# ruiminshen/yolo2-pytorch

Measured on NVIDIA H100. Metric: 416x416 images/sec, higher is better.
Workload: dtype f16

## Files before the change

yolo2-pytorch_b200/b200/engine.py:

```python
import os

import torch

from . import ops

STRICT_KEEP = {'layers1.0': 'aw', 'layers1.2': 'aw', 'layers1.4': 'a', 'passthrough': 'aw', 'layers3.0': 'aw'}
PRECISIONS = ('fast', 'strict')


class ConvUnit(object):

    def __init__(self, conv, bn, act):
        self.conv, self.bn, self.act = conv, bn, act
        self._wver = None
        self._bver = None
        self.w16 = self.scale = self.shift = None
        self.split_a = self.split_w = False
        self.out_lo = False

    @property
    def cout(self):
        return self.conv.weight.shape[0]

    @property
# ... 6 lines not shown

    @property
    def slope(self):
        return 0.1 if self.act else 1.0

    def refresh(self, first_layer=False, force=False):
        w = self.conv.weight
        wver = (w.data_ptr(), w._version)
        wver = wver + (self.split_a, self.split_w)
        if force or wver != self._wver:
            if first_layer:
                self.w16 = w.detach().contiguous()
            elif self.split_a or self.split_w:
                self.w16 = ops.pack_weight_split_f16(w.detach().contiguous(), self.split_a, self.split_w)
            else:
                self.w16 = ops.pack_weight_f16(w.detach().contiguous(), 0)
            self._wver = wver
        if self.bn is not None:
            ts = (self.bn.weight, self.bn.bias, self.bn.running_mean, self.bn.running_var)
            bver = tuple((t.data_ptr(), t._version) for t in ts)
            if bver != self._bver:
                self.scale, self.shift = ops.bn_fold(*(t.detach().contiguous() for t in ts), eps=self.bn.eps)
                self._bver = bver
        else:
            b = self.conv.bias
            bver = None if b is None else (b.data_ptr(), b._version)
            if bver != self._bver or self.scale is None:
                self.scale = torch.ones(self.cout, dtype=torch.float32, device=w.device)
                self.shift = (b.detach().float().contiguous().clone() if b is not None
                              else torch.zeros(self.cout, dtype=torch.float32, device=w.device))
                self._bver = bver


class StrictPlan(object):

    def __init__(self, eng, batch, height, width, device):
        f16 = dict(dtype=torch.float16, device=device)

        def buf(u, h, w):
            return torch.empty(batch, h, w, u.cout * (2 if u.out_lo else 1), **f16)

        h, w = height // 2, width // 2
        self.a0 = torch.empty(batch, h, w, eng.units1[0].cout, **f16)
        self.l1 = []
        for u, pooled in zip(eng.units1[1:], eng.pools1[1:]):
            out = buf(u, h, w)
            if pooled:
                h, w = h // 2, w // 2
                self.l1.append((out, buf(u, h, w)))
            else:
                self.l1.append((out, None))
        self.pt = buf(eng.unit_pt, h, w)
        h, w = h // 2, w // 2
        self.x1_pool = buf(eng.units1[-1], h, w)
        self.cat_c = eng.unit_pt.cout * 4 + eng.units2[-1].cout
        self.cat = torch.empty(batch, h, w, self.cat_c * (2 if eng.units3[0].split_a else 1), **f16)
        self.l2 = [buf(u, h, w) for u in eng.units2[:-1]]
        self.l3 = buf(eng.units3[0], h, w)
        self.feature = torch.empty(batch, eng.units3[1].cout, h, w, dtype=torch.float32, device=device)
        self.workspace = ops.conv_workspace(device)


class DarknetPlan(object):

    def __init__(self, units1, units2, unit_pt, units3, pools1, batch, height, width, device):
        f16 = dict(dtype=torch.float16, device=device)
        self.batch, self.height, self.width = batch, height, width
        h, w = height // 2, width // 2
        self.a0 = torch.empty(batch, h, w, units1[0].cout, **f16)
        self.l1 = []
        for u, pooled in zip(units1[1:], pools1[1:]):
            out = torch.empty(batch, h, w, u.cout, **f16)
            if pooled:
                h, w = h // 2, w // 2
                self.l1.append((out, torch.empty(batch, h, w, u.cout, **f16)))
            else:
                self.l1.append((out, None))
        self.h16, self.w16 = h, w
        self.pt = torch.empty(batch, h, w, unit_pt.cout, **f16)
        self.x1_pool = torch.empty(batch, h // 2, w // 2, units1[-1].cout, **f16)
        h, w = h // 2, w // 2
        self.h32, self.w32 = h, w
        self.cat_ch = unit_pt.cout * 4 + units2[-1].cout
        self.cat = torch.empty(batch, h, w, self.cat_ch, **f16)
        self.l2 = [torch.empty(batch, h, w, u.cout, **f16) for u in units2[:-1]]
        self.l3 = torch.empty(batch, h, w, units3[0].cout, **f16)
        self.feature = torch.empty(batch, units3[1].cout, h, w, dtype=torch.float32, device=device)
        self.workspace = ops.conv_workspace(device)


class DarknetEngine(object):
    def __init__(self, dnn):
        def unit(m):
            return ConvUnit(m.conv, m.bn if m.has_bn else None, m.has_act)

        self.units1, self.pools1, self._k1 = [], [], []
        mods = list(dnn.layers1)
        for i, m in enumerate(mods):
# ... 57 lines not shown

    def invalidate(self):
        for u in self.all_units():
            u._wver = None
            u._bver = None

    def forward(self, x, conv_flags=0, ref=False, collect=None, plan_id=0):
        if not x.is_cuda:
            raise RuntimeError('Darknet: input must be a CUDA tensor; there is no CPU fallback')
        u8 = x.dtype == torch.uint8
        if u8:
            b, h, w, c = x.shape
        else:
            b, c, h, w = x.shape
        if c != 3 or h % 32 or w % 32:
            raise ValueError('Darknet expects fp32 [B,3,H,W] or uint8 [B,H,W,3] with H, W multiples of 32, got %s' % (tuple(x.shape),))
        x = x.contiguous() if u8 else x.contiguous().float()
        self.refresh()
        p = self.plan(b, h, w, x.device, plan_id)
        if self.precision == 'strict':
            return self._forward_strict(x, u8, p, conv_flags, collect)

        def conv(u, src, dst, **kw):
            return ops.conv_bn_act(src, u.w16, u.scale, u.shift, u.slope, out=dst, flags=conv_flags, ref=ref, workspace=p.workspace, **kw)

        u0 = self.units1[0]
        conv0 = ops.conv0_u8_bn_leaky_pool if u8 else ops.conv0_bn_leaky_pool
        cur = conv0(x, u0.w16, u0.scale, u0.shift, u0.slope, out=p.a0)
        if collect is not None:
            collect['layers1.0(pooled)'] = cur
        x1 = None
        last1 = self.units1[-1]
        for u, (out, pooled), key in zip(self.units1[1:], p.l1, self._k1[1:]):
            fuse_pool = (pooled is not None and u is not last1 and collect is None and not ref and u.cin == 32 and u.ksize == 3
                         and u.cout <= 64 and (conv_flags & (ops.CONV_NO_SMALLK | ops.CONV_C32_IM2COL)) == 0 and conv_flags < 256)
            if fuse_pool:
                ops.conv_bn_act(cur, u.w16, u.scale, u.shift, u.slope, out=pooled, flags=conv_flags | ops.CONV_POOL2X2)
                cur = pooled
                continue
            conv(u, cur, out)
            if collect is not None:
                collect[key] = out
            x1 = out
            cur = ops.maxpool2x2(out, out=pooled) if pooled is not None else out
        conv(self.unit_pt, x1, p.pt)
        if collect is not None:
            collect['passthrough'] = p.pt
        ops.reorg_f16(p.pt, p.cat, 0)
        cur = ops.maxpool2x2(x1, out=p.x1_pool)
        for u, out, key in zip(self.units2[:-1], p.l2, self._k2):
            conv(u, cur, out)
            if collect is not None:
                collect[key] = out
            cur = out
        conv(self.units2[-1], cur, p.cat, y_ch_off=self.unit_pt.cout * 4)
        conv(self.units3[0], p.cat, p.l3)
        conv(self.units3[1], p.l3, p.feature, out_mode=ops.OUT_F32_NCHW)
        if collect is not None:
            collect['cat'] = p.cat
            collect['layers3.0'] = p.l3
        return p.feature

    def _forward_strict(self, x, u8, p, conv_flags, collect):
        def view(t, c, lo):
            return (t[..., :c].float() + t[..., c:2 * c].float()) if lo else t[..., :c]

        def conv(u, src, src_c, src_lo, dst, y_ch_off=0, lo_ch_off=None, out_mode=ops.OUT_F16_NHWC):
            split_a = u.split_a and src_lo
            if lo_ch_off is None:
                lo_ch_off = y_ch_off + u.cout if u.out_lo else -1
            if not (split_a or u.split_w or lo_ch_off >= 0):
                return ops.conv_bn_act(src, u.w16, u.scale, u.shift, u.slope, out=dst, flags=conv_flags, workspace=p.workspace, cin=src_c,
                                       y_ch_off=y_ch_off, out_mode=out_mode)
            if u.split_a and not src_lo:
                raise RuntimeError('strict plan: unit expects [hi | lo] input')
            return ops.conv_bn_act_split(src, u.w16, u.scale, u.shift, u.slope, dst, a_channels=src_c * (2 if split_a else 1), y_ch_off=y_ch_off,
                                         lo_ch_off=lo_ch_off, out_mode=out_mode, flags=conv_flags, workspace=p.workspace)

        u0 = self.units1[0]
        conv0 = ops.conv0_u8_bn_leaky_pool if u8 else ops.conv0_bn_leaky_pool
        cur, cur_c, cur_lo = conv0(x, u0.w16, u0.scale, u0.shift, u0.slope, out=p.a0), u0.cout, False
        if collect is not None:
            collect['layers1.0(pooled)'] = cur
        x1 = None
        for u, (out, pooled), key in zip(self.units1[1:], p.l1, self._k1[1:]):
            plain = not (u.split_a or u.split_w or u.out_lo)
            if (plain and pooled is not None and collect is None and u.cin == 32 and u.ksize == 3 and u.cout <= 64 and conv_flags == 0):
                ops.conv_bn_act(cur, u.w16, u.scale, u.shift, u.slope, out=pooled, flags=ops.CONV_POOL2X2)
                cur, cur_c, cur_lo = pooled, u.cout, False
                continue
            conv(u, cur, cur_c, cur_lo, out)
            if collect is not None:
                collect[key] = view(out, u.cout, u.out_lo)
            x1, x1_c, x1_lo = out, u.cout, u.out_lo
            cur, cur_c, cur_lo = out, u.cout, u.out_lo
            if pooled is not None:
                cur = ops.maxpool2x2_split(out, u.cout, pooled) if u.out_lo else ops.maxpool2x2(out, out=pooled)
        cat_lo = self.units3[0].split_a
        upt = self.unit_pt
        conv(upt, x1, x1_c, x1_lo, p.pt)
        if collect is not None:
            collect['passthrough'] = view(p.pt, upt.cout, upt.out_lo)
        ops.reorg_f16(p.pt, p.cat, 0, channels=upt.cout)
        if cat_lo:
            ops.reorg_f16(p.pt, p.cat, p.cat_c, channels=upt.cout, x_ch_off=upt.cout)
        last1 = self.units1[-1]
        cur = ops.maxpool2x2_split(x1, last1.cout, p.x1_pool) if last1.out_lo else ops.maxpool2x2(x1, out=p.x1_pool)
        cur_c, cur_lo = last1.cout, last1.out_lo
        for u, out, key in zip(self.units2[:-1], p.l2, self._k2):
            conv(u, cur, cur_c, cur_lo, out)
            if collect is not None:
                collect[key] = view(out, u.cout, u.out_lo)
            cur, cur_c, cur_lo = out, u.cout, u.out_lo
        u27 = self.units2[-1]
        conv(u27, cur, cur_c, cur_lo, p.cat, y_ch_off=upt.cout * 4, lo_ch_off=(p.cat_c + upt.cout * 4) if cat_lo else -1)
        u30, u31 = self.units3
        conv(u30, p.cat, p.cat_c, cat_lo, p.l3)
        conv(u31, p.l3, u30.cout, u30.out_lo, p.feature, out_mode=ops.OUT_F32_NCHW, lo_ch_off=-1)
        if collect is not None:
            collect['cat'] = view(p.cat, p.cat_c, cat_lo)
# ... 3 lines not shown
```

yolo2-pytorch_b200/b200/ops.py:

```python
import ctypes

import torch

from . import lib as _l

OUT_F16_NHWC, OUT_F32_NCHW = 0, 1
CONV_A_TILED, CONV_WIDE_N = 1, 2
CONV_NO_STREAMK, CONV_FORCE_STREAMK, CONV_NO_SMALLK, CONV_PLAIN_STORE = 8, 1 << 30, 1 << 28, 1 << 29
CONV_POOL2X2, CONV_C32_IM2COL, CONV_C32_SWAP = 16, 32, 64
FILTER_THRESHOLD, FILTER_FIX, FILTER_NONE = 0, 1, 2


launch_count = 0


def _ck(rc, what):
    global launch_count
    _l.check(rc, what)
    launch_count += 1


def conv_force_bn(bn):
    return bn << 8

# ... 75 lines not shown
def conv0_u8_bn_leaky_pool(x, w, scale, shift, slope, out=None):
    _req(x, torch.uint8, 'x'); _req(w, torch.float32, 'w'); _req(scale, torch.float32, 'scale'); _req(shift, torch.float32, 'shift')
    b, h, wd, c = x.shape
    if c != 3:
        raise ValueError('conv0 expects 3 input channels')
    cout = w.shape[0]
    if out is None:
        out = torch.empty(b, h // 2, wd // 2, cout, dtype=torch.float16, device=x.device)
    _req(out, torch.float16, 'out')
    _ck(_l.load().yb_conv0_u8_bn_leaky_pool_fwd(_p(x), _p(w), _p(scale), _p(shift), float(slope), _p(out), b, h, wd, cout, _s()),
        'yb_conv0_u8_bn_leaky_pool_fwd')
    return out


def _conv_common(fn_name, x, w, scale, shift, slope, out, batch, height, width, cin, cout, k, x_ld, y_ld, y_ch_off, out_mode, flags,
                 workspace=None):
    if workspace is not None and fn_name == 'yb_conv_bn_act_fwd':
        fn_name = 'yb_conv_bn_act_fwd_ws'
    fn = getattr(_l.load(), fn_name)
    args = [_p(x), _p(w), _p(scale), _p(shift), float(slope), _p(out), batch, height, width, cin, cout, k, x_ld, y_ld, y_ch_off, out_mode]
    if fn_name != 'yb_conv_ref_fwd':
        args.append(flags)
    if fn_name == 'yb_conv_bn_act_fwd_ws':
        _req(workspace, torch.uint8, 'workspace')
        args += [_p(workspace), workspace.numel()]
    args.append(_s())
    _ck(fn(*args), fn_name)


def conv_workspace(device='cuda'):
    return torch.zeros(int(_l.load().yb_conv_workspace_bytes()), dtype=torch.uint8, device=device)


CONV_KERNELS = ('conv_igemm_kernel', 'conv_wide_kernel', 'conv_c32_kernel')


def conv_choice(batch, height, width, cin, cout, k, out_mode=OUT_F16_NHWC, flags=0, workspace=True):
    out = (ctypes.c_int * 6)()
    _l.check(_l.load().yb_conv_choice(batch, height, width, cin, cout, k, out_mode, flags, int(bool(workspace)), ctypes.byref(out)),
             'yb_conv_choice')
    return dict(kernel=CONV_KERNELS[out[0]], bk=out[1], bn=out[2], rows=out[3], streamk=bool(out[4]), grid=out[5])


def conv_bn_act(x, w, scale, shift, slope, out=None, out_mode=OUT_F16_NHWC, y_ch_off=0, cin=None, flags=0, ref=False, workspace=None):
    _req(x, torch.float16, 'x'); _req(w, torch.float16, 'w'); _req(scale, torch.float32, 'scale'); _req(shift, torch.float32, 'shift')
    b, h, wd, x_ld = x.shape
    cout, k, _, wcin = w.shape
    cin = wcin if cin is None else cin
    if cin != wcin:
        raise ValueError('weight Cin %d != %d' % (wcin, cin))
    if out is None:
        oh, ow = (h // 2, wd // 2) if (flags & CONV_POOL2X2) else (h, wd)
        out = (torch.empty(b, oh, ow, cout, dtype=torch.float16, device=x.device) if out_mode == OUT_F16_NHWC
               else torch.empty(b, cout, h, wd, dtype=torch.float32, device=x.device))
    if out_mode == OUT_F16_NHWC:
        _req(out, torch.float16, 'out')
        y_ld = out.shape[-1]
    else:
        _req(out, torch.float32, 'out')
        y_ld = 0
    _conv_common('yb_conv_ref_fwd' if ref else 'yb_conv_bn_act_fwd', x, w, scale, shift, slope, out, b, h, wd, cin, cout, k, x_ld, y_ld,
                 y_ch_off, out_mode, flags, workspace=None if ref else workspace)
    return out


def conv_bn_act_split(x, w, scale, shift, slope, out, a_channels, y_ch_off=0, lo_ch_off=-1, out_mode=OUT_F16_NHWC, flags=0, workspace=None):
    _req(x, torch.float16, 'x'); _req(w, torch.float16, 'w'); _req(scale, torch.float32, 'scale'); _req(shift, torch.float32, 'shift')
    b, h, wd, x_ld = x.shape
    cout, k, _, kch = w.shape
    if out_mode == OUT_F16_NHWC:
        _req(out, torch.float16, 'out')
        y_ld = out.shape[-1]
    else:
        _req(out, torch.float32, 'out')
# ... 182 lines not shown
```

yolo2-pytorch_b200/csrc/conv_igemm.cu:

```cuda
#include "yb_common.h"
#include "yb_ptx.cuh"
#include <stdlib.h>

namespace yb {

struct ConvParams {
  int m_total;
  int height, width;
  int cin, cout;
  int ksize, pad;
  int kb_per_tap;
  int num_kb;
  int m_tiles, n_tiles;
  int a_im2col;
  const float* scale;
  const float* shift;
  float slope;
  void* y;
  long long y_ld;
  int y_ch_off;
  int out_mode;
  int hw;
  int skip;
  int* dbg;
// ... 921 lines not shown
          __half2 h2 = __floats2half2_rn(f[g * 8 + 4], f[g * 8 + 5]), h3 = __floats2half2_rn(f[g * 8 + 6], f[g * 8 + 7]);
          pk[half * 4 + g].x = *reinterpret_cast<uint32_t*>(&h0); pk[half * 4 + g].y = *reinterpret_cast<uint32_t*>(&h1);
          pk[half * 4 + g].z = *reinterpret_cast<uint32_t*>(&h2); pk[half * 4 + g].w = *reinterpret_cast<uint32_t*>(&h3);
        }
      }
      const uint32_t obuf = smem_o + (grp * 2 + (use & 1)) * Cfg::kOutBytes;
      if (gt == 0) tma_store_wait_read<1>();
      asm volatile("bar.sync %0, 128;" :: "r"(1 + grp) : "memory");
      if (et == 0) { YB_TRACE(2, tr); ++tr; }
      if (writer) {
#pragma unroll
        for (int c = 0; c < 8; ++c) st_shared_v4(obuf + srow * 128 + ((c ^ (srow & 7)) << 4), pk[c]);
      }
      fence_proxy_async_smem();
      asm volatile("bar.sync %0, 128;" :: "r"(1 + grp) : "memory");
      if (gt == 0 && !(p.skip & 8)) {
        if (p.pool) tma_store_4d(&tmap_y, obuf, 0, tw * (Cfg::TW / 2), th * (Cfg::TH / 2), n);
        else tma_store_4d(&tmap_y, obuf, 0, tw * Cfg::TW, th * Cfg::TH, n);
        tma_store_commit();
      }
      if (et == 0) { YB_TRACE(2, tr); ++tr; }
    }
    if (gt == 0) tma_store_wait<0>();
    if (p.stats != nullptr) {
      asm volatile("bar.sync 8, %0;" :: "n"(Cfg::kEpiThreads) : "memory");
      for (int i = et; i < p.cout; i += Cfg::kEpiThreads) {
        atomicAdd(p.stats + i, static_cast<double>(ep_stats[i]));
        atomicAdd(p.stats + p.cout + i, static_cast<double>(ep_stats[BN + i]));
      }
    }
  }
}

constexpr long long kSkFlagBytes = 4096;
constexpr long long kSkSlotBytes = kWideRows * kWideBN * 4;
long long conv_workspace_bytes() { return kSkFlagBytes + kSkSlotBytes * sm_count(); }

constexpr int kKernelIgemm = 0;
constexpr int kKernelWide = 1;
constexpr int kKernelC32 = 2;
struct ConvChoice {
  int kernel, bk, bn, mt, streamk, grid;
};

static unsigned long long* g_conv_trace = nullptr;
void conv_set_trace(void* dev_ptr) { g_conv_trace = static_cast<unsigned long long*>(dev_ptr); }

typedef CUresult (*EncodeTiledFn)(CUtensorMap*, CUtensorMapDataType, cuuint32_t, void*, const cuuint64_t*, const cuuint64_t*,
                                  const cuuint32_t*, const cuuint32_t*, CUtensorMapInterleave, CUtensorMapSwizzle,
                                  CUtensorMapL2promotion, CUtensorMapFloatOOBfill);
typedef CUresult (*EncodeIm2colFn)(CUtensorMap*, CUtensorMapDataType, cuuint32_t, void*, const cuuint64_t*, const cuuint64_t*,
                                   const int*, const int*, cuuint32_t, cuuint32_t, const cuuint32_t*, CUtensorMapInterleave,
                                   CUtensorMapSwizzle, CUtensorMapL2promotion, CUtensorMapFloatOOBfill);

static int get_encoders(EncodeTiledFn* tiled, EncodeIm2colFn* im2col) {
  static EncodeTiledFn s_tiled = nullptr;
  static EncodeIm2colFn s_im2col = nullptr;
  if (s_tiled == nullptr || s_im2col == nullptr) {
    void* f0 = nullptr;
    void* f1 = nullptr;
    cudaDriverEntryPointQueryResult q0, q1;
    YB_CUDA(cudaGetDriverEntryPoint("cuTensorMapEncodeTiled", &f0, cudaEnableDefault, &q0));
    YB_CUDA(cudaGetDriverEntryPoint("cuTensorMapEncodeIm2col", &f1, cudaEnableDefault, &q1));
    if (f0 == nullptr || f1 == nullptr || q0 != cudaDriverEntryPointSuccess || q1 != cudaDriverEntryPointSuccess)
      return fail(YB_ERR_DRIVER, "cuTensorMapEncode* driver entry points unavailable");
    s_tiled = reinterpret_cast<EncodeTiledFn>(f0);
    s_im2col = reinterpret_cast<EncodeIm2colFn>(f1);
  }
  *tiled = s_tiled;
  *im2col = s_im2col;
  return 0;
}

// ... 100 lines not shown
    cr = enc_tiled(&tx, CU_TENSOR_MAP_DATA_TYPE_FLOAT16, 4, const_cast<void*>(x), dims, strides, box, estr, CU_TENSOR_MAP_INTERLEAVE_NONE,
                   CU_TENSOR_MAP_SWIZZLE_NONE, CU_TENSOR_MAP_L2_PROMOTION_L2_128B, CU_TENSOR_MAP_FLOAT_OOB_FILL_NONE);
    if (cr != CUDA_SUCCESS) return fail(YB_ERR_DRIVER, "cuTensorMapEncodeTiled(halo) failed (%d)", static_cast<int>(cr));
  }
  {
    const cuuint64_t dims[2] = {9 * 32, static_cast<cuuint64_t>(cout)};
    const cuuint64_t strides[1] = {9 * 32 * 2};
    const cuuint32_t box[2] = {32, 64};
    const cuuint32_t estr[2] = {1, 1};
    cr = enc_tiled(&tw, CU_TENSOR_MAP_DATA_TYPE_FLOAT16, 2, const_cast<void*>(w), dims, strides, box, estr, CU_TENSOR_MAP_INTERLEAVE_NONE,
                   CU_TENSOR_MAP_SWIZZLE_64B, CU_TENSOR_MAP_L2_PROMOTION_L2_256B, CU_TENSOR_MAP_FLOAT_OOB_FILL_NONE);
    if (cr != CUDA_SUCCESS) return fail(YB_ERR_DRIVER, "cuTensorMapEncodeTiled(W) failed (%d)", static_cast<int>(cr));
  }
  {
    const int oh = pool ? height / 2 : height, ow = pool ? width / 2 : width;
    const cuuint64_t dims[4] = {static_cast<cuuint64_t>(cout), static_cast<cuuint64_t>(ow), static_cast<cuuint64_t>(oh), static_cast<cuuint64_t>(batch)};
    const cuuint64_t strides[3] = {static_cast<cuuint64_t>(y_ld) * 2, static_cast<cuuint64_t>(y_ld) * 2 * ow, static_cast<cuuint64_t>(y_ld) * 2 * ow * oh};
    const cuuint32_t box[4] = {64, static_cast<cuuint32_t>(pool ? Cfg::TW / 2 : Cfg::TW), static_cast<cuuint32_t>(pool ? Cfg::TH / 2 : Cfg::TH), 1};
    const cuuint32_t estr[4] = {1, 1, 1, 1};
    cr = enc_tiled(&ty, CU_TENSOR_MAP_DATA_TYPE_FLOAT16, 4, static_cast<__half*>(y) + y_ch_off, dims, strides, box, estr,
                   CU_TENSOR_MAP_INTERLEAVE_NONE, CU_TENSOR_MAP_SWIZZLE_128B, CU_TENSOR_MAP_L2_PROMOTION_NONE, CU_TENSOR_MAP_FLOAT_OOB_FILL_NONE);
    if (cr != CUDA_SUCCESS) return fail(YB_ERR_DRIVER, "cuTensorMapEncodeTiled(Y) failed (%d)", static_cast<int>(cr));
  }
  static bool attr_set = false;
  if (!attr_set) {
    YB_CUDA(cudaFuncSetAttribute(conv_c32_kernel, cudaFuncAttributeMaxDynamicSharedMemorySize, Cfg::kSmemBytes));
    attr_set = true;
  }
  const int grid = p.num_tiles < sm_count() ? p.num_tiles : sm_count();
  conv_c32_kernel<<<grid, Cfg::kThreads, Cfg::kSmemBytes, stream>>>(tx, tw, ty, p);
  return check_launch("conv_c32_kernel");
}

constexpr double kKbNsIm2col = 240.0;
constexpr double kKbNsTiled = 100.0;
constexpr double kFeedBytesPerNs = 130.0;
constexpr double kEpiNsPerOut = 0.15;
constexpr double kWideEpiNsPerOut = 0.08;
constexpr double kSkNs = 16000.0;
constexpr double kSkNsWide = 9000.0;
int conv_choose(int batch, int height, int width, int cin, int cout, int ksize, int a_channels, int out_mode, int flags, bool workspace_ok,
                bool stats, bool lo, ConvChoice* out) {
  ConvChoice c;
  memset(&c, 0, sizeof(c));
  const int sms = sm_count();
  const bool split = a_channels != cin || lo;
  if (!split && cin == 32 && ksize == 3 && cout <= 64 && out_mode == 0 && ((flags >> 28) & 1) == 0 && ((flags >> 5) & 1) == 0 && ((flags >> 8) & 0xFFFF) == 0) {
    const long long tiles = static_cast<long long>(batch) * ((width + C32Cfg::TW - 1) / C32Cfg::TW) * ((height + C32Cfg::TH - 1) / C32Cfg::TH);
    c.kernel = kKernelC32; c.bk = 32; c.bn = C32Cfg::BN; c.mt = 1;
    c.grid = static_cast<int>(tiles < sms ? tiles : sms);
    *out = c;
    return 0;
  }
  if ((flags >> 4) & 1) return fail(YB_ERR_UNSUPPORTED, "conv: YB_CONV_POOL2X2 is only implemented for the Cin = 32 3x3 layer");
  const int bk = (cin % 64 == 0 && a_channels % 64 == 0) ? 64 : 32;
  const bool sk_possible = !stats && workspace_ok && (flags & 8) == 0;
  const bool sk_force = sk_possible && ((flags >> 30) & 1);
  const bool wide_ok = out_mode == 0 && !lo && !stats && ((flags >> 24) & 0xF) == 0 && ((flags >> 29) & 1) == 0;
  const int force_bn = (flags >> 8) & 0x3FF;
  const int force_mt = (flags >> 20) & 0x3;
  const int force_pair = (flags >> 22) & 0x3;
  YB_REQUIRE(force_pair != 2, "conv: CTA-pair tiles need two-CTA tensor-core instructions, which sm_90 does not have");
  YB_REQUIRE(!force_bn || ((force_bn == 64 || force_bn == 128) && (force_mt != 2 || force_bn == 64 || wide_ok)),
             "conv: BLOCK_N=%d x %d M-subtiles is not a tile shape of this launch (64 x 1, 128 x 1, 64 x 2; 128 x 2 for fp16 NHWC "
             "outputs without residual or statistics)", force_bn, force_mt ? force_mt : 1);
  const long long m_total = static_cast<long long>(batch) * height * width;
  const int num_kb = ksize * ksize * (cin / bk);
  double best = 1e300;
  for (int cbn = 64; cbn <= 128; cbn *= 2) {
    if (force_bn && cbn != force_bn) continue;
    if (!force_bn && cbn > 64 && cbn / 2 >= cout) continue;
    for (int cmt = 1; cmt <= 2; ++cmt) {
      if (force_mt && cmt != force_mt) continue;
      const bool cwide = cmt * cbn > 128;
      if (cwide && !wide_ok) continue;
      const int rows_tile = BM * cmt;
      const double tiles = static_cast<double>((m_total + rows_tile - 1) / rows_tile) * ((cout + cbn - 1) / cbn);
      const double rounds = static_cast<double>((static_cast<long long>(tiles) + sms - 1) / sms);
      const double kb_ns = (ksize == 3 ? kKbNsIm2col : kKbNsTiled) + (cmt * BM + cbn) * bk * 2.0 / kFeedBytesPerNs;
      const double main_ns = num_kb * kb_ns;
      const double outs = static_cast<double>(rows_tile) * cbn;
      const double tile_ns = cwide ? main_ns + outs * kWideEpiNsPerOut : (main_ns > outs * kEpiNsPerOut ? main_ns : outs * kEpiNsPerOut);
      double t = rounds * tile_ns;
      int csk = 0;
      if (sk_possible) {
        const double units = tiles * num_kb;
        const double per_cta = static_cast<double>((static_cast<long long>(units) + sms - 1) / sms);
        const double tsk = per_cta * kb_ns + (cwide ? kSkNsWide : kSkNs);
        const bool ok = per_cta >= 4.0 && num_kb >= 2;
        const bool idle = tiles <= sms / 2;
        if (ok && (sk_force || (idle && tsk < 0.93 * t))) { t = tsk; csk = 1; }
      }
      if (sk_force && !csk) continue;
      if (t < best * 0.9999 || (t <= best * 1.0001 && cbn > c.bn)) { best = t; c.bn = cbn; c.mt = cmt; c.streamk = csk; }
    }
  }
  if (c.bn == 0) { c.bn = force_bn ? force_bn : 128; c.mt = force_mt ? force_mt : 1; c.streamk = 0; }
  YB_REQUIRE((c.bn == 64 || c.bn == 128) && (c.mt == 1 || c.mt == 2) && (c.mt * c.bn <= 128 || wide_ok), "conv: tile %d x %d", c.bn, c.mt);
  c.kernel = c.mt * c.bn > 128 ? kKernelWide : kKernelIgemm;
  c.bk = bk;
  const long long tiles = ((m_total + BM * c.mt - 1) / (BM * c.mt)) * ((cout + c.bn - 1) / c.bn);
  c.grid = c.streamk ? sms : static_cast<int>(tiles < sms ? tiles : sms);
  *out = c;
  return 0;
}

int conv_choice(int batch, int height, int width, int cin, int cout, int ksize, int out_mode, int flags, int with_workspace, int* out) {
  YB_REQUIRE(out != nullptr && batch > 0 && height > 0 && width > 0 && cin % 32 == 0 && cout > 0 && (ksize == 1 || ksize == 3),
             "conv_choice: bad shape");
  ConvChoice c;
  const int rc = conv_choose(batch, height, width, cin, cout, ksize, cin, out_mode, flags, with_workspace != 0, false, false, &c);
  if (rc) return rc;
  out[0] = c.kernel; out[1] = c.bk; out[2] = c.bn; out[3] = c.kernel == kKernelC32 ? C32Cfg::TH * C32Cfg::TW : BM * c.mt;
  out[4] = c.streamk; out[5] = c.grid;
  return 0;
}

int conv_igemm_forward(const void* x, const void* w, const float* scale, const float* shift, float slope, void* y, int batch,
                       int height, int width, int cin, int cout, int ksize, int x_ld, long long y_ld, int y_ch_off, int out_mode,
                       int flags, void* workspace, long long workspace_bytes, double* stats, int a_channels, int lo_ch_off, cudaStream_t stream) {
  YB_REQUIRE(x && w && scale && shift && y, "conv: null pointer");
  if (a_channels <= 0) a_channels = cin;
  YB_REQUIRE(a_channels <= cin && a_channels % 32 == 0 && cin - a_channels <= a_channels, "conv: a_channels=%d does not fit cin=%d", a_channels, cin);
  YB_REQUIRE(lo_ch_off < 0 || (out_mode == 0 && stats == nullptr && lo_ch_off % 8 == 0 && lo_ch_off >= y_ch_off + cout && lo_ch_off + cout <= y_ld),
             "conv: lo_ch_off=%d (needs fp16 NHWC output with room for a second Cout-wide slice)", lo_ch_off);
  YB_REQUIRE(stats == nullptr || out_mode == 0, "conv: fused statistics need the fp16 NHWC output");
  YB_REQUIRE(ksize == 1 || ksize == 3, "conv: ksize %d unsupported (1 or 3)", ksize);
  YB_REQUIRE(batch > 0 && height > 0 && width > 0, "conv: bad shape");
  YB_REQUIRE(cin % 32 == 0, "conv: Cin=%d must be a multiple of 32 (layer 0 uses yb_conv0_*)", cin);
  YB_REQUIRE(x_ld >= a_channels && x_ld % 8 == 0, "conv: x_ld=%d", x_ld);
  YB_REQUIRE((reinterpret_cast<uintptr_t>(x) & 15) == 0 && (reinterpret_cast<uintptr_t>(w) & 15) == 0, "conv: x/w must be 16B aligned");
  YB_REQUIRE(out_mode == 0 || out_mode == 1, "conv: out_mode");
  if (out_mode == 0) {
    YB_REQUIRE(cout % 8 == 0 && y_ld % 8 == 0 && y_ch_off % 8 == 0 && (reinterpret_cast<uintptr_t>(y) & 15) == 0,
               "conv: fp16 NHWC output needs Cout, y_ld, y_ch_off multiples of 8 and a 16B aligned pointer");
  }
  const long long m_total_ll = static_cast<long long>(batch) * height * width;
  YB_REQUIRE(m_total_ll < (1ll << 31) - kWideRows, "conv: too many pixels");
  const bool ws_ok = workspace != nullptr && workspace_bytes >= conv_workspace_bytes() && (reinterpret_cast<uintptr_t>(workspace) & 255) == 0;
  ConvChoice ch;
  int rc = conv_choose(batch, height, width, cin, cout, ksize, a_channels, out_mode, flags, ws_ok, stats != nullptr, lo_ch_off >= 0, &ch);
  if (rc) return rc;
  if (ch.kernel == kKernelC32)
    return conv_c32_forward(x, w, scale, shift, slope, y, batch, height, width, cout, x_ld, y_ld, y_ch_off, (flags >> 4) & 1, flags, stats, stream);
  const int bk = ch.bk, bn = ch.bn, mt = ch.mt, streamk = ch.streamk;
  static const int k1x1_im2col = getenv("YB_CONV_1X1_IM2COL") ? atoi(getenv("YB_CONV_1X1_IM2COL")) : 0;
  const int a_im2col = (ksize == 3) ? 1 : ((k1x1_im2col && !(flags & 1)) ? 1 : 0);

  EncodeTiledFn enc_tiled;
  EncodeIm2colFn enc_im2col;
  rc = get_encoders(&enc_tiled, &enc_im2col);
  if (rc) return rc;

  ConvParams p;
  p.m_total = static_cast<int>(m_total_ll);
  p.height = height; p.width = width; p.cin = cin; p.cout = cout; p.ksize = ksize; p.pad = (ksize - 1) / 2;
  p.kb_per_tap = cin / bk;
  p.num_kb = ksize * ksize * p.kb_per_tap;
  const int rows_tile = BM * mt;
  p.m_tiles = (p.m_total + rows_tile - 1) / rows_tile;
  p.n_tiles = (cout + bn - 1) / bn;
  p.a_im2col = a_im2col;
  p.scale = scale; p.shift = shift; p.slope = slope;
  p.y = y; p.y_ld = y_ld; p.y_ch_off = y_ch_off; p.out_mode = out_mode;
  p.hw = height * width;
  p.dbg = debug_word_device();
  p.trace = g_conv_trace;
  p.skip = (flags >> 24) & 0xF;
  p.streamk = streamk;
  p.stats = stats;
  p.tma_store = 0;
  p.a_wrap = a_channels;
  p.lo_off = lo_ch_off >= 0 ? static_cast<long long>(lo_ch_off - y_ch_off) : 0;
  p.sk_base = 0; p.sk_rem = 0; p.ws = nullptr; p.flags = nullptr;
  if (streamk) {
    const long long units = static_cast<long long>(p.m_tiles) * p.n_tiles * p.num_kb;
    YB_REQUIRE(units < (1ll << 31), "conv: stream-K unit count overflows");
// ... 111 lines not shown
```

yolo2-pytorch_b200/model/yolo2.py:

```python
import torch
import torch.nn as nn

import model
from b200 import engine as _engine
from b200 import ops as _ops
from b200 import train_engine as _train

settings = {
    'size': (416, 416),
}


def reorg(x, stride_h=2, stride_w=2):
    return _ops.reorg_f32_nchw(x.contiguous().float(), stride_h, stride_w)


class MaxPool2d(nn.Module):
    is_pool = True

    def __init__(self, kernel_size=2):
        nn.Module.__init__(self)
        if kernel_size != 2:
            raise ValueError('only MaxPool2d(2) is on the Darknet path')
        self.kernel_size = kernel_size
# ... 156 lines not shown
        self.padding = tuple(padding)


class MaxPool2dStride1(nn.Module):
    is_pool = True

    def __init__(self):
        nn.Module.__init__(self)
        self.kernel_size, self.stride = 2, 1


class Tiny(nn.Module):

    def __init__(self, config_channels, anchors, num_cls, channels=16):
        nn.Module.__init__(self)
        cc = config_channels
        bn = cc.config.getboolean('batch_norm', 'enable')
        layers = []
        for _ in range(5):
            layers.append(Conv2d(cc.channels, cc(channels, 'layers.%d.conv.weight' % len(layers)), 3, bn=bn, padding=True))
            layers.append(MaxPool2d(2))
            channels *= 2
        layers.append(Conv2d(cc.channels, cc(channels, 'layers.%d.conv.weight' % len(layers)), 3, bn=bn, padding=True))
        layers.append(ConstantPad2d((0, 1, 0, 1)))
        layers.append(MaxPool2dStride1())
        channels *= 2
        for _ in range(2):
            layers.append(Conv2d(cc.channels, cc(channels, 'layers.%d.conv.weight' % len(layers)), 3, bn=bn, padding=True))
        layers.append(Conv2d(cc.channels, model.output_channels(len(anchors), num_cls), 1, bn=False, act=False))
        self.layers = nn.Sequential(*layers)
        self.init()
        self._units = None
        self._pad_cache = {}
        self._trainer = None

    @property
    def trainer(self):
        if self._trainer is None:
            self._trainer = _train.TinyTrainer(self)
        return self._trainer

    def unit_keys(self):
        keys = ['layers.%d' % i for i, m in enumerate(self.layers) if not m.is_pool]
        return [(k, u, after) for k, (u, after) in zip(keys, self._plan())]

    def train(self, mode=True):
        if getattr(self, '_units', None) is not None and bool(mode) != self.training:
            self._pad_cache = {}
            for u, _ in self._units:
                u._wver = u._bver = None
        return nn.Module.train(self, mode)

    def init(self):
        for m in self.modules():
            if isinstance(m, nn.Conv2d):
                nn.init.xavier_normal_(m.weight)
            elif isinstance(m, nn.BatchNorm2d):
                nn.init.ones_(m.weight)
                nn.init.zeros_(m.bias)

    def scope(self, name):
        return '.'.join(name.split('.')[:-2])

    def _plan(self):
        if self._units is None:
            mods = list(self.layers)
# ... 22 lines not shown
        w_op = wp.contiguous() if first else _ops.pack_weight_f16(wp.contiguous(), 0)
        scale = torch.zeros(cout_to, dtype=torch.float32, device=w.device)
        shift = torch.zeros(cout_to, dtype=torch.float32, device=w.device)
        scale[:cout], shift[:cout] = u.scale, u.shift
        self._pad_cache[key] = (ver, (w_op, scale, shift))
        return self._pad_cache[key][1]

    def forward(self, x):
        if self.training:
            return _DarknetTrainFunction.apply(self, x, *[p for _, p in self.named_parameters()])
        if not x.is_cuda:
            raise RuntimeError('Tiny: input must be a CUDA tensor; there is no CPU fallback')
        b, c, h, w = x.shape
        if c != 3 or h % 32 or w % 32:
            raise ValueError('Tiny expects fp32 [B,3,H,W] with H, W multiples of 32, got %s' % (tuple(x.shape),))
        x = x.contiguous().float()
        plan = self._plan()
        for i, (u, _) in enumerate(plan):
            u.refresh(first_layer=(i == 0))
        u0, after0 = plan[0]
        if after0 != 'pool' or u0.cout > 32:
            raise RuntimeError('Tiny: the first unit must have <= 32 filters and be followed by MaxPool2d(2)')
        w0, sc0, sh0 = self._padded('u0', u0, 32, 3, True)
        cur = _ops.conv0_bn_leaky_pool(x, w0, sc0, sh0, u0.slope)
        chan = 32
        for i, (u, after) in enumerate(plan[1:], 1):
            last = i == len(plan) - 1
            if u.cin != chan:
                w_op, scale, shift = self._padded('u%d' % i, u, u.cout, chan, False)
            else:
                w_op, scale, shift = u.w16, u.scale, u.shift
            if last:
                return _ops.conv_bn_act(cur, w_op, scale, shift, u.slope, out_mode=_ops.OUT_F32_NCHW)
            fuse = after == 'pool' and chan == 32 and u.ksize == 3 and u.cout <= 64
            if fuse:
                cur = _ops.conv_bn_act(cur, w_op, scale, shift, u.slope, flags=_ops.CONV_POOL2X2)
            else:
                cur = _ops.conv_bn_act(cur, w_op, scale, shift, u.slope)
                if after == 'pool':
                    cur = _ops.maxpool2x2(cur)
                elif after == 'pool_s1':
                    cur = _ops.maxpool2x2_s1(cur)
            chan = u.cout
```

Baseline: 14430.

## Add halo-tile WGMMA conv kernel for Cin=64 3x3 layers with fused maxpool

Adds a new warp-specialized conv kernel for 3x3 layers with 64 input and 65-128 output channels. It TMA-loads 8x8 spatial tiles with a 1-pixel halo once and reuses them across all nine taps via WGMMA, with resident weights and a 3-stage pipeline. It can fuse the following 2x2 maxpool into the epilogue. The dispatcher selects it automatically, and the Python side now asks the C++ chooser whether pool fusion is supported rather than hardcoding Cin=32. This is meant to cut im2col/feed overhead and a separate maxpool pass on the 64->128 layer, at the cost of added complexity and a separate epilogue path.

Result: no change. 14610 (median of 6 runs) (+1.3%).

```diff
diff --git a/yolo2-pytorch_b200/b200/engine.py b/yolo2-pytorch_b200/b200/engine.py
--- a/yolo2-pytorch_b200/b200/engine.py
+++ b/yolo2-pytorch_b200/b200/engine.py
@@ -62,9 +62,22 @@
                 self._bver = bver
 
 
-class StrictPlan(object):
+class _Plan(object):
+    def __init__(self):
+        self._fuses_pool = {}
+
+    def fuses_pool(self, key, x, u, conv_flags):
+        k = (key, conv_flags)
+        if k not in self._fuses_pool:
+            b, h, w, _ = x.shape
+            self._fuses_pool[k] = ops.conv_fuses_pool(b, h, w, u.cin, u.cout, u.ksize, conv_flags)
+        return self._fuses_pool[k]
+
+
+class StrictPlan(_Plan):
 
     def __init__(self, eng, batch, height, width, device):
+        super(StrictPlan, self).__init__()
         f16 = dict(dtype=torch.float16, device=device)
 
         def buf(u, h, w):
@@ -91,9 +104,10 @@
         self.workspace = ops.conv_workspace(device)
 
 
-class DarknetPlan(object):
+class DarknetPlan(_Plan):
 
     def __init__(self, units1, units2, unit_pt, units3, pools1, batch, height, width, device):
+        super(DarknetPlan, self).__init__()
         f16 = dict(dtype=torch.float16, device=device)
         self.batch, self.height, self.width = batch, height, width
         h, w = height // 2, width // 2
@@ -217,9 +231,7 @@
         x1 = None
         last1 = self.units1[-1]
         for u, (out, pooled), key in zip(self.units1[1:], p.l1, self._k1[1:]):
-            fuse_pool = (pooled is not None and u is not last1 and collect is None and not ref and u.cin == 32 and u.ksize == 3
-                         and u.cout <= 64 and (conv_flags & (ops.CONV_NO_SMALLK | ops.CONV_C32_IM2COL)) == 0 and conv_flags < 256)
-            if fuse_pool:
+            if pooled is not None and u is not last1 and collect is None and not ref and p.fuses_pool(key, cur, u, conv_flags):
                 ops.conv_bn_act(cur, u.w16, u.scale, u.shift, u.slope, out=pooled, flags=conv_flags | ops.CONV_POOL2X2)
                 cur = pooled
                 continue
@@ -270,7 +282,7 @@
         x1 = None
         for u, (out, pooled), key in zip(self.units1[1:], p.l1, self._k1[1:]):
             plain = not (u.split_a or u.split_w or u.out_lo)
-            if (plain and pooled is not None and collect is None and u.cin == 32 and u.ksize == 3 and u.cout <= 64 and conv_flags == 0):
+            if plain and pooled is not None and collect is None and conv_flags == 0 and p.fuses_pool(key, cur, u, 0):
                 ops.conv_bn_act(cur, u.w16, u.scale, u.shift, u.slope, out=pooled, flags=ops.CONV_POOL2X2)
                 cur, cur_c, cur_lo = pooled, u.cout, False
                 continue
diff --git a/yolo2-pytorch_b200/b200/ops.py b/yolo2-pytorch_b200/b200/ops.py
--- a/yolo2-pytorch_b200/b200/ops.py
+++ b/yolo2-pytorch_b200/b200/ops.py
@@ -131,7 +131,7 @@
     return torch.zeros(int(_l.load().yb_conv_workspace_bytes()), dtype=torch.uint8, device=device)
 
 
-CONV_KERNELS = ('conv_igemm_kernel', 'conv_wide_kernel', 'conv_c32_kernel')
+CONV_KERNELS = ('conv_igemm_kernel', 'conv_wide_kernel', 'conv_c32_kernel', 'conv_halo_kernel')
 
 
 def conv_choice(batch, height, width, cin, cout, k, out_mode=OUT_F16_NHWC, flags=0, workspace=True):
@@ -139,6 +139,14 @@
     _l.check(_l.load().yb_conv_choice(batch, height, width, cin, cout, k, out_mode, flags, int(bool(workspace)), ctypes.byref(out)),
              'yb_conv_choice')
     return dict(kernel=CONV_KERNELS[out[0]], bk=out[1], bn=out[2], rows=out[3], streamk=bool(out[4]), grid=out[5])
+
+
+def conv_fuses_pool(batch, height, width, cin, cout, k, flags=0):
+    try:
+        conv_choice(batch, height, width, cin, cout, k, flags=flags | CONV_POOL2X2)
+    except RuntimeError:
+        return False
+    return True
 
 
 def conv_bn_act(x, w, scale, shift, slope, out=None, out_mode=OUT_F16_NHWC, y_ch_off=0, cin=None, flags=0, ref=False, workspace=None):
diff --git a/yolo2-pytorch_b200/csrc/conv_igemm.cu b/yolo2-pytorch_b200/csrc/conv_igemm.cu
--- a/yolo2-pytorch_b200/csrc/conv_igemm.cu
+++ b/yolo2-pytorch_b200/csrc/conv_igemm.cu
@@ -977,6 +977,180 @@
   }
 }
 
+struct HaloParams {
+  int blocks_w, blocks_h, num_blocks, num_tiles, cout;
+  const float* scale;
+  const float* shift;
+  float slope;
+  int pool;
+  int* dbg;
+};
+
+struct HaloCfg {
+  static constexpr int TB = 8, HB = TB + 2;
+  static constexpr int kPlaneData = HB * HB * 16;
+  static constexpr int kPlane = (kPlaneData + 127) / 128 * 128;
+  static constexpr int kBlock = 8 * kPlane;
+  static constexpr int kStage = 2 * kBlock;
+  static constexpr int kStages = 3;
+  static constexpr int BN = 128;
+  static constexpr int kBTap = BN * 64 * 2;
+  static constexpr int kBBytes = 9 * kBTap;
+  static constexpr int kOutBytes = 128 * 128;
+  static constexpr int kThreads = 384;
+  static constexpr int kSmemBytes = 1024  + kBBytes + kStages * kStage + 256 ;
+  static_assert(kSmemBytes <= kSmemLimit, "halo: shared memory budget");
+  static_assert(kOutBytes <= kStage && kStage % 1024 == 0 && kBBytes % 1024 == 0, "halo: the 128B-swizzled staging aliases a stage");
+};
+
+__device__ __forceinline__ void halo_block(const HaloParams& p, int blk, int& bx, int& by, int& n) {
+  bx = blk % p.blocks_w;
+  const int rest = blk / p.blocks_w;
+  by = rest % p.blocks_h;
+  n = rest / p.blocks_h;
+}
+
+__global__ void __launch_bounds__(HaloCfg::kThreads, 1)
+conv_halo_kernel(const __grid_constant__ CUtensorMap tmap_x, const __grid_constant__ CUtensorMap tmap_w,
+                 const __grid_constant__ CUtensorMap tmap_y, const HaloParams p) {
+  using Cfg = HaloCfg;
+  extern __shared__ uint8_t smem_raw[];
+  const uint32_t smem_base = (smem_u32(smem_raw) + 1023u) & ~1023u;
+  const uint32_t smem_b = smem_base;
+  const uint32_t smem_h = smem_b + Cfg::kBBytes;
+  const uint32_t bar_full = smem_h + Cfg::kStages * Cfg::kStage;
+  const uint32_t bar_empty = bar_full + 8 * Cfg::kStages;
+  const uint32_t bar_w = bar_empty + 8 * Cfg::kStages;
+
+  if (threadIdx.x == 0) {
+    for (int i = 0; i < Cfg::kStages; ++i) {
+      mbar_init(bar_full + 8 * i, 1);
+      mbar_init(bar_empty + 8 * i, 1);
+    }
+    mbar_init(bar_w, 1);
+    fence_mbar_init();
+    fence_proxy_async_smem();
+    tma_prefetch_desc(&tmap_x);
+    tma_prefetch_desc(&tmap_w);
+    tma_prefetch_desc(&tmap_y);
+  }
+  __syncthreads();
+  pdl_trigger();
+  pdl_wait();
+
+  if (threadIdx.x < 128) {
+    setmaxnreg_dec<40>();
+    if (threadIdx.x == 0) {
+      mbar_arrive_expect_tx(bar_w, Cfg::kBBytes);
+      for (int t = 0; t < 9; ++t) tma_load_2d(smem_b + t * Cfg::kBTap, &tmap_w, bar_w, t * 64, 0);
+      int local = 0;
+      for (int tile = blockIdx.x; tile < p.num_tiles; tile += gridDim.x, ++local) {
+        const int stage = local % Cfg::kStages;
+        mbar_wait(bar_empty + 8 * stage, ((local / Cfg::kStages) & 1) ^ 1, p.dbg, 0xC00 | stage);
+        const int nblk = 2 * tile + 1 < p.num_blocks ? 2 : 1;
+        const uint32_t full = bar_full + 8 * stage;
+        mbar_arrive_expect_tx(full, nblk * 8 * Cfg::kPlaneData);
+        for (int h = 0; h < nblk; ++h) {
+          int bx, by, n;
+          halo_block(p, 2 * tile + h, bx, by, n);
+          for (int c = 0; c < 8; ++c)
+            tma_load_4d(smem_h + stage * Cfg::kStage + h * Cfg::kBlock + c * Cfg::kPlane, &tmap_x, full, c * 8, bx * Cfg::TB - 1, by * Cfg::TB - 1, n);
+        }
+      }
+    }
+    return;
+  }
+  setmaxnreg_inc<232>();
+  const int cw = (threadIdx.x >> 7) - 1;
+  const int t = threadIdx.x & 127;
+  const int warp = t >> 5;
+  const int lane = t & 31;
+  float acc[2][64];
+  mbar_wait(bar_w, 0, p.dbg, 0xC10);
+  for (int tile = blockIdx.x + cw * gridDim.x, local = cw; tile < p.num_tiles; tile += 2 * gridDim.x, local += 2) {
+    const int stage = local % Cfg::kStages;
+    mbar_wait(bar_full + 8 * stage, (local / Cfg::kStages) & 1, p.dbg, 0xC20 | stage);
+    const uint32_t halo = smem_h + stage * Cfg::kStage;
+    wgmma_fence();
+#pragma unroll
+    for (int tap = 0; tap < 9; ++tap) {
+      const uint64_t bdesc = make_kmajor_desc<128>(smem_b + tap * Cfg::kBTap);
+      const uint32_t win = halo + ((tap / 3) * Cfg::HB + tap % 3) * 16;
+#pragma unroll
+      for (int h = 0; h < 2; ++h)
+#pragma unroll
+        for (int k = 0; k < 4; ++k)
+          wgmma_f16<Cfg::BN>(acc[h], make_kmajor_desc_noswz(win + h * Cfg::kBlock + 2 * k * Cfg::kPlane, Cfg::kPlane, Cfg::HB * 16),
+                             bdesc + 2 * k, (tap | k) != 0);
+    }
+    wgmma_commit();
+    wgmma_wait<0>();
+    fence_regs(acc[0]);
+    fence_regs(acc[1]);
+
+    const int nblk = 2 * tile + 1 < p.num_blocks ? 2 : 1;
+#pragma unroll
+    for (int c2 = 0; c2 < 2; ++c2) {
+      if (t == 0) tma_store_wait_read<0>();
+      asm volatile("bar.sync %0, 128;" :: "r"(2 + cw) : "memory");
+#pragma unroll
+      for (int jj = 0; jj < 8; ++jj) {
+        const int col = c2 * 64 + 8 * jj + 2 * (lane & 3);
+        const bool ok = col < p.cout;
+        const float sc0 = ok ? __ldg(p.scale + col) : 0.f, sc1 = ok ? __ldg(p.scale + col + 1) : 0.f;
+        const float sh0 = ok ? __ldg(p.shift + col) : 0.f, sh1 = ok ? __ldg(p.shift + col + 1) : 0.f;
+        const int j = c2 * 8 + jj;
+#pragma unroll
+        for (int h = 0; h < 2; ++h) {
+          float v[2][2];
+#pragma unroll
+          for (int hh = 0; hh < 2; ++hh) {
+            float x0 = acc[h][4 * j + 2 * hh] * sc0 + sh0;
+            float x1 = acc[h][4 * j + 2 * hh + 1] * sc1 + sh1;
+            v[hh][0] = x0 > 0.f ? x0 : x0 * p.slope;
+            v[hh][1] = x1 > 0.f ? x1 : x1 * p.slope;
+          }
+          if (p.pool) {
+            float m0 = fmaxf(v[0][0], v[1][0]), m1 = fmaxf(v[0][1], v[1][1]);
+            m0 = fmaxf(m0, __shfl_xor_sync(0xffffffffu, m0, 4));
+            m1 = fmaxf(m1, __shfl_xor_sync(0xffffffffu, m1, 4));
+            if ((lane & 4) == 0) {
+              __half2 hv = __floats2half2_rn(m0, m1);
+              const int r = h * 16 + warp * 4 + (lane >> 3);
+              const uint32_t addr = halo + r * 128 + ((jj ^ (r & 7)) << 4) + 4 * (lane & 3);
+              asm volatile("st.shared.b32 [%0], %1;" :: "r"(addr), "r"(*reinterpret_cast<uint32_t*>(&hv)) : "memory");
+            }
+          } else {
+#pragma unroll
+            for (int hh = 0; hh < 2; ++hh) {
+              __half2 hv = __floats2half2_rn(v[hh][0], v[hh][1]);
+              const int r = h * 64 + warp * 16 + (lane >> 2) + hh * 8;
+              const uint32_t addr = halo + r * 128 + ((jj ^ (r & 7)) << 4) + 4 * (lane & 3);
+              asm volatile("st.shared.b32 [%0], %1;" :: "r"(addr), "r"(*reinterpret_cast<uint32_t*>(&hv)) : "memory");
+            }
+          }
+        }
+      }
+      fence_proxy_async_smem();
+      asm volatile("bar.sync %0, 128;" :: "r"(2 + cw) : "memory");
+      if (t == 0) {
+        for (int h = 0; h < nblk; ++h) {
+          int bx, by, n;
+          halo_block(p, 2 * tile + h, bx, by, n);
+          if (p.pool) tma_store_4d(&tmap_y, halo + h * 16 * 128, c2 * 64, bx * (Cfg::TB / 2), by * (Cfg::TB / 2), n);
+          else tma_store_4d(&tmap_y, halo + h * 64 * 128, c2 * 64, bx * Cfg::TB, by * Cfg::TB, n);
+        }
+        tma_store_commit();
+      }
+    }
+    if (t == 0) {
+      tma_store_wait_read<0>();
+      mbar_arrive(bar_empty + 8 * stage);
+    }
+  }
+  if (t == 0) tma_store_wait<0>();
+}
+
 constexpr long long kSkFlagBytes = 4096;
 constexpr long long kSkSlotBytes = kWideRows * kWideBN * 4;
 long long conv_workspace_bytes() { return kSkFlagBytes + kSkSlotBytes * sm_count(); }
@@ -984,6 +1158,7 @@
 constexpr int kKernelIgemm = 0;
 constexpr int kKernelWide = 1;
 constexpr int kKernelC32 = 2;
+constexpr int kKernelHalo = 3;
 struct ConvChoice {
   int kernel, bk, bn, mt, streamk, grid;
 };
@@ -1150,6 +1325,65 @@
   return check_launch("conv_c32_kernel");
 }
 
+static int conv_halo_forward(const void* x, const void* w, const float* scale, const float* shift, float slope, void* y, int batch,
+                             int height, int width, int cout, int x_ld, long long y_ld, int y_ch_off, int pool, cudaStream_t stream) {
+  using Cfg = HaloCfg;
+  EncodeTiledFn enc_tiled;
+  EncodeIm2colFn enc_im2col;
+  int rc = get_encoders(&enc_tiled, &enc_im2col);
+  if (rc) return rc;
+  HaloParams p;
+  p.blocks_w = width / Cfg::TB;
+  p.blocks_h = height / Cfg::TB;
+  const long long nb = static_cast<long long>(batch) * p.blocks_w * p.blocks_h;
+  YB_REQUIRE(nb < (1ll << 30), "conv: too many tiles");
+  p.num_blocks = static_cast<int>(nb);
+  p.num_tiles = (p.num_blocks + 1) / 2;
+  p.cout = cout;
+  p.scale = scale; p.shift = shift; p.slope = slope;
+  p.pool = pool;
+  p.dbg = debug_word_device();
+  alignas(64) CUtensorMap tx, tw, ty;
+  CUresult cr;
+  {
+    const cuuint64_t dims[4] = {64, static_cast<cuuint64_t>(width), static_cast<cuuint64_t>(height), static_cast<cuuint64_t>(batch)};
+    const cuuint64_t strides[3] = {static_cast<cuuint64_t>(x_ld) * 2, static_cast<cuuint64_t>(x_ld) * 2 * width,
+                                   static_cast<cuuint64_t>(x_ld) * 2 * width * height};
+    const cuuint32_t box[4] = {8, Cfg::HB, Cfg::HB, 1};
+    const cuuint32_t estr[4] = {1, 1, 1, 1};
+    cr = enc_tiled(&tx, CU_TENSOR_MAP_DATA_TYPE_FLOAT16, 4, const_cast<void*>(x), dims, strides, box, estr, CU_TENSOR_MAP_INTERLEAVE_NONE,
+                   CU_TENSOR_MAP_SWIZZLE_NONE, CU_TENSOR_MAP_L2_PROMOTION_L2_128B, CU_TENSOR_MAP_FLOAT_OOB_FILL_NONE);
+    if (cr != CUDA_SUCCESS) return fail(YB_ERR_DRIVER, "cuTensorMapEncodeTiled(halo) failed (%d)", static_cast<int>(cr));
+  }
+  {
+    const cuuint64_t dims[2] = {9 * 64, static_cast<cuuint64_t>(cout)};
+    const cuuint64_t strides[1] = {9 * 64 * 2};
+    const cuuint32_t box[2] = {64, Cfg::BN};
+    const cuuint32_t estr[2] = {1, 1};
+    cr = enc_tiled(&tw, CU_TENSOR_MAP_DATA_TYPE_FLOAT16, 2, const_cast<void*>(w), dims, strides, box, estr, CU_TENSOR_MAP_INTERLEAVE_NONE,
+                   CU_TENSOR_MAP_SWIZZLE_128B, CU_TENSOR_MAP_L2_PROMOTION_L2_256B, CU_TENSOR_MAP_FLOAT_OOB_FILL_NONE);
+    if (cr != CUDA_SUCCESS) return fail(YB_ERR_DRIVER, "cuTensorMapEncodeTiled(W) failed (%d)", static_cast<int>(cr));
+  }
+  {
+    const int oh = pool ? height / 2 : height, ow = pool ? width / 2 : width, ob = pool ? Cfg::TB / 2 : Cfg::TB;
+    const cuuint64_t dims[4] = {static_cast<cuuint64_t>(cout), static_cast<cuuint64_t>(ow), static_cast<cuuint64_t>(oh), static_cast<cuuint64_t>(batch)};
+    const cuuint64_t strides[3] = {static_cast<cuuint64_t>(y_ld) * 2, static_cast<cuuint64_t>(y_ld) * 2 * ow, static_cast<cuuint64_t>(y_ld) * 2 * ow * oh};
+    const cuuint32_t box[4] = {64, static_cast<cuuint32_t>(ob), static_cast<cuuint32_t>(ob), 1};
+    const cuuint32_t estr[4] = {1, 1, 1, 1};
+    cr = enc_tiled(&ty, CU_TENSOR_MAP_DATA_TYPE_FLOAT16, 4, static_cast<__half*>(y) + y_ch_off, dims, strides, box, estr,
+                   CU_TENSOR_MAP_INTERLEAVE_NONE, CU_TENSOR_MAP_SWIZZLE_128B, CU_TENSOR_MAP_L2_PROMOTION_NONE, CU_TENSOR_MAP_FLOAT_OOB_FILL_NONE);
+    if (cr != CUDA_SUCCESS) return fail(YB_ERR_DRIVER, "cuTensorMapEncodeTiled(Y) failed (%d)", static_cast<int>(cr));
+  }
+  static bool attr_set = false;
+  if (!attr_set) {
+    YB_CUDA(cudaFuncSetAttribute(conv_halo_kernel, cudaFuncAttributeMaxDynamicSharedMemorySize, Cfg::kSmemBytes));
+    attr_set = true;
+  }
+  const int grid = p.num_tiles < sm_count() ? p.num_tiles : sm_count();
+  conv_halo_kernel<<<grid, Cfg::kThreads, Cfg::kSmemBytes, stream>>>(tx, tw, ty, p);
+  return check_launch("conv_halo_kernel");
+}
+
 constexpr double kKbNsIm2col = 240.0;
 constexpr double kKbNsTiled = 100.0;
 constexpr double kFeedBytesPerNs = 130.0;
@@ -1170,7 +1404,16 @@
     *out = c;
     return 0;
   }
-  if ((flags >> 4) & 1) return fail(YB_ERR_UNSUPPORTED, "conv: YB_CONV_POOL2X2 is only implemented for the Cin = 32 3x3 layer");
+  const bool forced = ((flags >> 8) & 0xFFFF) != 0 || ((flags >> 24) & 0x7F) != 0;
+  if (!split && !stats && cin == 64 && ksize == 3 && cout > 64 && cout <= 128 && out_mode == 0 && height % HaloCfg::TB == 0 &&
+      width % HaloCfg::TB == 0 && !forced) {
+    const long long tiles = (static_cast<long long>(batch) * (height / HaloCfg::TB) * (width / HaloCfg::TB) + 1) / 2;
+    c.kernel = kKernelHalo; c.bk = 64; c.bn = HaloCfg::BN; c.mt = 1;
+    c.grid = static_cast<int>(tiles < sms ? tiles : sms);
+    *out = c;
+    return 0;
+  }
+  if ((flags >> 4) & 1) return fail(YB_ERR_UNSUPPORTED, "conv: YB_CONV_POOL2X2 is only implemented for the 3x3 Cin = 32 and Cin = 64 halo-tile layers");
   const int bk = (cin % 64 == 0 && a_channels % 64 == 0) ? 64 : 32;
   const bool sk_possible = !stats && workspace_ok && (flags & 8) == 0;
   const bool sk_force = sk_possible && ((flags >> 30) & 1);
@@ -1229,7 +1472,7 @@
   ConvChoice c;
   const int rc = conv_choose(batch, height, width, cin, cout, ksize, cin, out_mode, flags, with_workspace != 0, false, false, &c);
   if (rc) return rc;
-  out[0] = c.kernel; out[1] = c.bk; out[2] = c.bn; out[3] = c.kernel == kKernelC32 ? C32Cfg::TH * C32Cfg::TW : BM * c.mt;
+  out[0] = c.kernel; out[1] = c.bk; out[2] = c.bn; out[3] = c.kernel == kKernelC32 ? C32Cfg::TH * C32Cfg::TW : c.kernel == kKernelHalo ? 2 * 64 : BM * c.mt;
   out[4] = c.streamk; out[5] = c.grid;
   return 0;
 }
@@ -1261,6 +1504,8 @@
   if (rc) return rc;
   if (ch.kernel == kKernelC32)
     return conv_c32_forward(x, w, scale, shift, slope, y, batch, height, width, cout, x_ld, y_ld, y_ch_off, (flags >> 4) & 1, flags, stats, stream);
+  if (ch.kernel == kKernelHalo)
+    return conv_halo_forward(x, w, scale, shift, slope, y, batch, height, width, cout, x_ld, y_ld, y_ch_off, (flags >> 4) & 1, stream);
   const int bk = ch.bk, bn = ch.bn, mt = ch.mt, streamk = ch.streamk;
   static const int k1x1_im2col = getenv("YB_CONV_1X1_IM2COL") ? atoi(getenv("YB_CONV_1X1_IM2COL")) : 0;
   const int a_im2col = (ksize == 3) ? 1 : ((k1x1_im2col && !(flags & 1)) ? 1 : 0);
diff --git a/yolo2-pytorch_b200/model/yolo2.py b/yolo2-pytorch_b200/model/yolo2.py
--- a/yolo2-pytorch_b200/model/yolo2.py
+++ b/yolo2-pytorch_b200/model/yolo2.py
@@ -212,6 +212,7 @@
         self.init()
         self._units = None
         self._pad_cache = {}
+        self._fuse_cache = {}
         self._trainer = None
 
     @property
@@ -300,7 +301,12 @@
                 w_op, scale, shift = u.w16, u.scale, u.shift
             if last:
                 return _ops.conv_bn_act(cur, w_op, scale, shift, u.slope, out_mode=_ops.OUT_F32_NCHW)
-            fuse = after == 'pool' and chan == 32 and u.ksize == 3 and u.cout <= 64
+            fuse = False
+            if after == 'pool':
+                key = (i,) + tuple(cur.shape)
+                if key not in self._fuse_cache:
+                    self._fuse_cache[key] = _ops.conv_fuses_pool(cur.shape[0], cur.shape[1], cur.shape[2], chan, u.cout, u.ksize)
+                fuse = self._fuse_cache[key]
             if fuse:
                 cur = _ops.conv_bn_act(cur, w_op, scale, shift, u.slope, flags=_ops.CONV_POOL2X2)
             else:
```
